# Champii/raiko

Measured on AMD Instinct MI355X. Metric: proven RISC-V cycles/sec, higher is better.
Workload: dtype u32 (BabyBear Montgomery)

## Files before the change

### include/raiko_hip.h

```cpp
#ifndef RAIKO_HIP_H
#define RAIKO_HIP_H
#include <stddef.h>
#include <stdint.h>

#ifdef __cplusplus
extern "C" {
#endif

typedef enum {
    RK_OK = 0,
    RK_ERR_INVALID = -1,
    RK_ERR_HIP = -2,
    RK_ERR_NOMEM = -3,
    RK_ERR_NODEVICE = -4,
    RK_ERR_CAPACITY = -5,
    RK_ERR_INTERNAL = -6,
    RK_ERR_VERIFY = -7,
    RK_ERR_CALLBACK = -8
} rk_status;

typedef struct rk_ctx rk_ctx;

int rk_abi_version(void);
const char* rk_strerror(int status);
// ... 179 lines not shown

typedef struct {
    int device;
    int inflight;
    int upload_ahead;
    int verify;
    const int* devices;
    int n_devices;
    const rk_verify_opts* verify_opts;
    const rk_params* params;
} rk_session_opts;
int rk_prove_session(const rk_session_opts* opts, const rk_segment* segs, size_t n, uint32_t* const* h_seals,
                     const size_t* seal_capacity_words, size_t* seal_words, size_t* failed_index);
typedef struct rk_stream rk_stream;
int rk_stream_open(const rk_session_opts* opts, rk_stream** out);
int rk_stream_submit(rk_stream* stream, const rk_segment* seg, uint32_t* h_seal, size_t seal_capacity_words, size_t* seal_words);
int rk_stream_wait(rk_stream* stream, size_t max_pending, size_t* finished_prefix);
int rk_stream_close(rk_stream* stream, size_t* failed_index);
const char* rk_session_last_error(int device);
int rk_session_last_proven(int device, size_t* count);
int rk_session_release(void);
int rk_code_cache_configure(int device, size_t max_bytes);
int rk_code_cache_stats(int device, uint64_t* hits, uint64_t* misses, uint64_t* bytes);

typedef struct rk_comm rk_comm;
#define RK_COMM_ID_BYTES 128
int rk_comm_unique_id(uint8_t id[RK_COMM_ID_BYTES]);
int rk_comm_create(const uint8_t id[RK_COMM_ID_BYTES], int rank, int world, int device, rk_comm** out);
int rk_comm_destroy(rk_comm* comm);
const char* rk_comm_last_error(rk_comm* comm);
int rk_gather_seals(rk_comm* comm, const uint32_t* const* h_local_seals, const size_t* local_words, size_t n_local, size_t n_total,
                    uint32_t* const* h_out, const size_t* out_capacity, size_t* out_words);
int rk_gather_unpack(const uint32_t* all_lens, const uint32_t* all_payload, int world, size_t per_rank, size_t max_len, size_t n_total,
                     uint32_t* const* h_out, const size_t* out_capacity, size_t* out_words);

typedef struct rk_exec rk_exec;
enum { RK_ECALL_HALT = 0, RK_ECALL_READ = 1, RK_ECALL_COMMIT = 2 };
enum { RK_EXIT_HALTED = 0, RK_EXIT_SYSTEM_SPLIT = 2 };
typedef struct {
    uint32_t struct_size;
    uint32_t segment_limit_po2;
    uint64_t session_limit;
    const uint32_t* input_words;
    size_t n_input_words;
    uint32_t record_trace;
    uint32_t profile;
// ... 334 lines not shown
```

### provers/hip/driver/src/ffi.rs

```rust
#![allow(non_camel_case_types)]
#![allow(clippy::missing_safety_doc)]
use std::os::raw::{c_char, c_int, c_void};
pub const RK_ECALL_HALT: c_int = 0;
pub const RK_ECALL_READ: c_int = 1;
pub const RK_ECALL_COMMIT: c_int = 2;

pub const RK_EXIT_HALTED: c_int = 0;
pub const RK_EXIT_SYSTEM_SPLIT: c_int = 2;

pub type rk_status = c_int;
pub const RK_OK: rk_status = 0;
pub const RK_ERR_INVALID: rk_status = -1;
pub const RK_ERR_HIP: rk_status = -2;
pub const RK_ERR_NOMEM: rk_status = -3;
pub const RK_ERR_NODEVICE: rk_status = -4;
pub const RK_ERR_CAPACITY: rk_status = -5;
pub const RK_ERR_INTERNAL: rk_status = -6;
pub const RK_ERR_VERIFY: rk_status = -7;
pub const RK_ERR_CALLBACK: rk_status = -8;

pub type rk_preset = c_int;
pub const RK_PRESET_RISC0: rk_preset = 0;
pub const RK_PRESET_SP1: rk_preset = 1;

// ... 218 lines not shown
#[repr(C)]
#[derive(Clone, Copy)]
pub struct rk_verify_opts {
    pub p2_rc_ext: *const u32,
    pub p2_rc_int: *const u32,
    pub p2_diag: *const u32,
    pub poly_ext: Option<rk_poly_ext_fn>,
    pub user: *mut c_void,
    pub program: *const rk_program,
    pub params: *const rk_params,
}

#[repr(C)]
#[derive(Clone, Copy)]
pub struct rk_session_opts {
    pub device: c_int,
    pub inflight: c_int,
    pub upload_ahead: c_int,
    pub verify: c_int,
    pub devices: *const c_int,
    pub n_devices: c_int,
    pub verify_opts: *const rk_verify_opts,
    pub params: *const rk_params,
}

#[repr(C)]
#[derive(Clone, Copy)]
pub struct rk_exec_opts {
    pub struct_size: u32,
    pub segment_limit_po2: u32,
    pub session_limit: u64,
    pub input_words: *const u32,
    pub n_input_words: usize,
    pub record_trace: u32,
    pub profile: u32,
}

#[repr(C)]
#[derive(Clone, Copy)]
pub struct rk_exec_summary {
    pub total_cycles: u64,
    pub n_segments: u32,
    pub exit_code: u32,
    pub journal_bytes: usize,
    pub input_words_read: usize,
    pub status: c_int,
// ... 287 lines not shown
    pub fn rk_program_create(steps: *const rk_poly_step, n_steps: usize, ret: u32, taps: *const rk_taps, out: *mut *mut rk_program) -> c_int;
    pub fn rk_program_destroy(prog: *mut rk_program) -> c_int;
    pub fn rk_program_get_info(prog: *const rk_program, out: *mut rk_program_info) -> c_int;
    pub fn rk_program_eval_check(prog: *const rk_program, view: *const rk_circuit_view, poly_mix: *const u32, d_check: *mut u32) -> c_int;
    pub fn rk_program_compile(prog: *mut rk_program, ctx: *mut rk_ctx) -> c_int;
    pub fn rk_program_source(prog: *const rk_program, out: *mut c_char, capacity: usize, length: *mut usize) -> c_int;
    pub fn rk_program_poly_ext(prog: *const rk_program, ext_w: u32, poly_mix: *const u32, eval_u_ext: *const u32, n_taps: usize, globals: *const u32, n_globals: u32, mix: *const u32, n_mix: u32, out_ext: *mut u32) -> c_int;
    pub fn rk_prove_segment(ctx: *mut rk_ctx, seg: *const rk_segment, h_seal: *mut u32, seal_capacity_words: usize, seal_words: *mut usize) -> c_int;
    pub fn rk_verify_segment(pub_: *const rk_segment, seal: *const u32, seal_words: usize) -> c_int;
    pub fn rk_verify_segment_ex(pub_: *const rk_segment, opts: *const rk_verify_opts, seal: *const u32, seal_words: usize) -> c_int;
    pub fn rk_seal_bound_words(seg: *const rk_segment) -> usize;
    pub fn rk_seal_bound_words_for(seg: *const rk_segment, queries: u32) -> usize;
    pub fn rk_seal_bound_words_params(seg: *const rk_segment, params: *const rk_params) -> usize;
    pub fn rk_prove_session(opts: *const rk_session_opts, segs: *const rk_segment, n: usize, h_seals: *const *mut u32, seal_capacity_words: *const usize, seal_words: *mut usize, failed_index: *mut usize) -> c_int;
    pub fn rk_stream_open(opts: *const rk_session_opts, out: *mut *mut rk_stream) -> c_int;
    pub fn rk_stream_submit(stream: *mut rk_stream, seg: *const rk_segment, h_seal: *mut u32, seal_capacity_words: usize, seal_words: *mut usize) -> c_int;
    pub fn rk_stream_wait(stream: *mut rk_stream, max_pending: usize, finished_prefix: *mut usize) -> c_int;
    pub fn rk_stream_close(stream: *mut rk_stream, failed_index: *mut usize) -> c_int;
    pub fn rk_session_last_error(device: c_int) -> *const c_char;
    pub fn rk_session_last_proven(device: c_int, count: *mut usize) -> c_int;
    pub fn rk_session_release() -> c_int;
    pub fn rk_code_cache_configure(device: c_int, max_bytes: usize) -> c_int;
    pub fn rk_code_cache_stats(device: c_int, hits: *mut u64, misses: *mut u64, bytes: *mut u64) -> c_int;
    pub fn rk_comm_unique_id(id: *mut u8) -> c_int;
    pub fn rk_comm_create(id: *const u8, rank: c_int, world: c_int, device: c_int, out: *mut *mut rk_comm) -> c_int;
    pub fn rk_comm_destroy(comm: *mut rk_comm) -> c_int;
    pub fn rk_comm_last_error(comm: *mut rk_comm) -> *const c_char;
    pub fn rk_gather_seals(comm: *mut rk_comm, h_local_seals: *const *const u32, local_words: *const usize, n_local: usize, n_total: usize, h_out: *const *mut u32, out_capacity: *const usize, out_words: *mut usize) -> c_int;
    pub fn rk_gather_unpack(all_lens: *const u32, all_payload: *const u32, world: c_int, per_rank: usize, max_len: usize, n_total: usize, h_out: *const *mut u32, out_capacity: *const usize, out_words: *mut usize) -> c_int;
    pub fn rk_exec_elf(elf: *const u8, elf_bytes: usize, opts: *const rk_exec_opts, out: *mut *mut rk_exec) -> c_int;
    pub fn rk_exec_open(elf: *const u8, elf_bytes: usize, opts: *const rk_exec_opts, out: *mut *mut rk_exec) -> c_int;
    pub fn rk_exec_next_segment(ex: *mut rk_exec, more: *mut c_int) -> c_int;
    pub fn rk_exec_summary_get(ex: *const rk_exec, out: *mut rk_exec_summary) -> c_int;
    pub fn rk_exec_segment_get(ex: *const rk_exec, index: u32, out: *mut rk_exec_segment) -> c_int;
    pub fn rk_exec_journal(ex: *const rk_exec, out: *mut u8, capacity: usize, len: *mut usize) -> c_int;
    pub fn rk_exec_profile(ex: *const rk_exec, pcs: *mut u32, cycles: *mut u64, capacity: usize, n: *mut usize) -> c_int;
    pub fn rk_exec_witness(ex: *const rk_exec, index: u32, code: *mut u32, data: *mut u32) -> c_int;
    pub fn rk_exec_lookup_tables(ex: *const rk_exec, index: u32, range_table: *mut u32, program_table: *mut u32, program_rows: *mut usize) -> c_int;
    pub fn rk_exec_witness_device(ctx: *mut rk_ctx, ex: *const rk_exec, index: u32, d_code: *mut u32, d_data: *mut u32) -> c_int;
    pub fn rk_exec_witness_device_rows(ctx: *mut rk_ctx, ex: *const rk_exec, index: u32, d_rows: *mut u32) -> c_int;
    pub fn rk_exec_registers(ex: *const rk_exec, index: u32, start: *mut u32, end: *mut u32) -> c_int;
    pub fn rk_exec_ecalls(ex: *const rk_exec, index: u32, out: *mut u32, capacity: usize, n: *mut usize) -> c_int;
    pub fn rk_exec_rv32_sizes(ex: *const rk_exec, index: u32, program_rows: *mut usize) -> c_int;
    pub fn rk_exec_rv32_shard_device(ctx: *mut rk_ctx, ex: *const rk_exec, index: u32, d_cpu: *mut u32, d_program: *mut u32, program_rows: usize, d_register: *mut u32, d_byte: *mut u32, d_range: *mut u32) -> c_int;
    pub fn rk_exec_rv32cf_shard_device(ctx: *mut rk_ctx, ex: *const rk_exec, index: u32, d_cpu: *mut u32, d_program: *mut u32, program_rows: usize, d_register: *mut u32, d_byte: *mut u32, d_range: *mut u32, d_shift: *mut u32) -> c_int;
    pub fn rk_exec_rv32im_sizes(ex: *const rk_exec, index: u32, muldiv_rows: *mut usize) -> c_int;
// ... 80 lines not shown
```

### raiko_amd/_lib.py

```python
import ctypes as C
import os

_HERE = os.path.dirname(os.path.abspath(__file__))
LIB_PATH = os.environ.get("RAIKO_HIP_LIB") or os.path.join(_HERE, "libraiko_hip.so")


class HipLibraryError(RuntimeError):
    pass


class RkError(RuntimeError):
    def __init__(self, status, detail=""):
        self.status = status
        super().__init__(f"libraiko_hip status {status}: {detail}")


u32p = C.POINTER(C.c_uint32)


class RkTaps(C.Structure):
    _fields_ = [
        ("group_size", C.c_uint32 * 3),
        ("n_regs", C.c_uint32),
        ("reg_group", u32p),
# ... 63 lines not shown

class RkVerifyOpts(C.Structure):
    _fields_ = [("p2_rc_ext", u32p), ("p2_rc_int", u32p), ("p2_diag", u32p), ("poly_ext", POLY_EXT_FN),
                ("user", C.c_void_p), ("program", C.c_void_p), ("params", C.POINTER(RkParams))]


class RkSessionOpts(C.Structure):
    _fields_ = [("device", C.c_int), ("inflight", C.c_int), ("upload_ahead", C.c_int), ("verify", C.c_int),
                ("devices", C.POINTER(C.c_int)), ("n_devices", C.c_int), ("verify_opts", C.POINTER(RkVerifyOpts)),
                ("params", C.POINTER(RkParams))]


RK_ERR_INVALID = -1
RK_ERR_CAPACITY = -5
RK_ERR_INTERNAL = -6
RK_ERR_VERIFY = -7
RK_ERR_CALLBACK = -8


class RkKernelStat(C.Structure):
    _fields_ = [("launches", C.c_uint64), ("ms", C.c_double), ("bytes", C.c_double)]


KCLASS_COUNT = 5


class RkTiming(C.Structure):
    _fields_ = [(n, C.c_float) for n in ("ntt", "hash", "deep", "fri", "query", "total", "circuit")]


class RkFriReduceSizeInfo(C.Structure):
    _fields_ = [(n, C.c_uint32) for n in ("n_rounds", "n_slots", "fold_width", "path_width", "reduce_width", "chip_width", "fold_log_height",
                                          "path_log_height", "reduce_log_height", "chip_log_height")] + \
               [(n, C.c_uint64) for n in ("fold_rows", "path_rows", "reduce_rows", "chip_rows", "rows_per_query", "fold_publics_words",
                                          "fold_records_words", "reduce_publics_words", "inputs_words")]


class RkFriOpenSizeInfo(C.Structure):
    _fields_ = [(n, C.c_uint32) for n in ("n_rounds", "n_slots", "n_groups", "n_batches", "log_pmax", "log_kmax", "fold_width", "path_width",
                                          "reduce_width", "ipath_width", "chip_width", "state_width", "fold_log_height", "path_log_height",
                                          "reduce_log_height", "ipath_log_height", "chip_log_height", "state_log_height")] + \
               [(n, C.c_uint64) for n in ("fold_rows", "path_rows", "reduce_rows", "ipath_rows", "chip_rows", "state_rows", "rows_per_query",
                                          "fold_publics_words", "fold_records_words", "reduce_publics_words", "inputs_words", "roots_words",
                                          "paths_words")]


# ... 50 lines not shown
class RkExecSummary(C.Structure):
    _fields_ = [("total_cycles", C.c_uint64), ("n_segments", C.c_uint32), ("exit_code", C.c_uint32),
                ("journal_bytes", C.c_size_t), ("input_words_read", C.c_size_t), ("status", C.c_int)]


class RkExecSegment(C.Structure):
    _fields_ = [("index", C.c_uint32), ("po2", C.c_uint32), ("cycles", C.c_uint64), ("start_pc", C.c_uint32),
                ("end_pc", C.c_uint32), ("exit", C.c_uint32), ("pre_state", C.c_uint32 * 8), ("post_state", C.c_uint32 * 8)]


_vp, _sz, _u32 = C.c_void_p, C.c_size_t, C.c_uint32
SYMBOLS = {
    "rk_prove_session": (C.c_int, [C.POINTER(RkSessionOpts), C.POINTER(RkSegment), _sz, C.POINTER(u32p), C.POINTER(_sz),
                                   C.POINTER(_sz), C.POINTER(_sz)]),
    "rk_session_last_error": (C.c_char_p, [C.c_int]),
    "rk_stream_open": (C.c_int, [C.POINTER(RkSessionOpts), C.POINTER(C.c_void_p)]),
    "rk_stream_submit": (C.c_int, [C.c_void_p, C.POINTER(RkSegment), u32p, C.c_size_t, C.POINTER(C.c_size_t)]),
    "rk_stream_wait": (C.c_int, [C.c_void_p, C.c_size_t, C.POINTER(C.c_size_t)]),
    "rk_stream_close": (C.c_int, [C.c_void_p, C.POINTER(C.c_size_t)]),
    "rk_session_release": (C.c_int, []),
    "rk_session_last_proven": (C.c_int, [C.c_int, C.POINTER(C.c_size_t)]),
    "rk_code_cache_configure": (C.c_int, [C.c_int, C.c_size_t]),
    "rk_code_cache_stats": (C.c_int, [C.c_int, C.POINTER(C.c_uint64), C.POINTER(C.c_uint64), C.POINTER(C.c_uint64)]),
    "rk_abi_version": (C.c_int, []),
    "rk_strerror": (C.c_char_p, [C.c_int]),
    "rk_last_error": (C.c_char_p, [_vp]),
    "rk_device_count": (C.c_int, [C.POINTER(C.c_int)]),
    "rk_ctx_create": (C.c_int, [C.c_int, _vp, C.POINTER(_vp)]),
    "rk_ctx_destroy": (C.c_int, [_vp]),
    "rk_sync": (C.c_int, [_vp]),
    "rk_alloc": (C.c_int, [_vp, _sz, C.POINTER(_vp)]),
    "rk_free": (C.c_int, [_vp, _vp]),
    "rk_h2d": (C.c_int, [_vp, _vp, _vp, _sz]),
    "rk_d2h": (C.c_int, [_vp, _vp, _vp, _sz]),
    "rk_set_poseidon2_params": (C.c_int, [_vp, u32p, u32p, u32p]),
    "rk_batch_interpolate_ntt": (C.c_int, [_vp, _vp, _sz, _sz]),
    "rk_batch_evaluate_ntt": (C.c_int, [_vp, _vp, _sz, _sz, _u32]),
    "rk_zk_shift": (C.c_int, [_vp, _vp, _sz, _sz]),
    "rk_batch_expand_into_evaluate_ntt": (C.c_int, [_vp, _vp, _vp, _sz, _sz, _u32]),
    "rk_batch_bit_reverse": (C.c_int, [_vp, _vp, _sz, _sz]),
    "rk_hash_rows": (C.c_int, [_vp, _vp, _vp, _sz, _sz]),
    "rk_hash_fold": (C.c_int, [_vp, _vp, _sz, _sz]),
    "rk_batch_evaluate_any": (C.c_int, [_vp, _vp, _sz, _sz, u32p, u32p, _sz, u32p]),
    "rk_mix_poly_coeffs": (C.c_int, [_vp, _vp, u32p, u32p, _vp, u32p, _sz, _sz]),
    "rk_eltwise_add_elem": (C.c_int, [_vp, _vp, _vp, _vp, _sz]),
    "rk_eltwise_sum_extelem": (C.c_int, [_vp, _vp, _vp, _sz, _sz]),
# ... 205 lines not shown
```

### raiko_amd/csrc/code_cache.hip

```cpp
#include "internal.hpp"

#include <cstdlib>
#include <list>
#include <mutex>
#include <random>

namespace rk {

namespace {

constexpr unsigned FP_CHUNK = 4096;
constexpr unsigned FP_TPB = 256;
constexpr unsigned FP_PER_LANE = FP_CHUNK / FP_TPB;
constexpr size_t FP_MAX_CHUNKS = (size_t)1 << 16;
constexpr unsigned FP_MAX_BLOCKS = 1024;
constexpr unsigned FP_PART = 8;

__global__ __launch_bounds__(FP_TPB) void code_fingerprint_kernel(uint32_t* __restrict__ part, const uint32_t* __restrict__ m,
                                                                  size_t words, const uint32_t* __restrict__ ta,
                                                                  const uint32_t* __restrict__ tb, uint32_t wm, int vec) {
    const unsigned t = threadIdx.x;
    uint32_t a[FP_PER_LANE][4];
#pragma unroll
    for (unsigned q = 0; q < 4; q++)
// ... 38 lines not shown
        tot = bb::add(tot, bb::mul(s, bb::Ext{{bv.x, bv.y, bv.z, bv.w}}, wm));
    }
    __shared__ uint32_t red[FP_TPB][5];
#pragma unroll
    for (unsigned c = 0; c < 4; c++) red[t][c] = tot.c[c];
    red[t][4] = bad;
    __syncthreads();
    for (unsigned h = FP_TPB / 2; h > 0; h >>= 1) {
        if (t < h) {
#pragma unroll
            for (unsigned c = 0; c < 4; c++) red[t][c] = bb::add(red[t][c], red[t + h][c]);
            red[t][4] |= red[t + h][4];
        }
        __syncthreads();
    }
    if (t < 5) part[(size_t)blockIdx.x * FP_PART + t] = red[0][t];
}

struct DevCache {
    std::mutex mu;
    std::list<std::shared_ptr<CodeEntry>> lru;
    size_t bytes = 0, max_bytes = 0;
    uint64_t hits = 0, misses = 0;
    uint32_t* d_tables = nullptr;
};

std::mutex g_mu;
std::map<int, DevCache*>* g_caches = nullptr;

size_t default_bytes() {
    static const size_t v = [] {
        const char* e = std::getenv("RK_CODE_CACHE_BYTES");
        if (e && *e) return (size_t)std::strtoull(e, nullptr, 0);
        return (size_t)2 << 30;
    }();
    return v;
}

DevCache* cache_of(int device) {
    std::lock_guard<std::mutex> l(g_mu);
    if (!g_caches) g_caches = new std::map<int, DevCache*>();
    DevCache*& c = (*g_caches)[device];
    if (!c) {
        c = new DevCache();
        c->max_bytes = default_bytes();
    }
// ... 78 lines not shown
    for (int i = 0; i < 4; i++) fp[i] = sum.c[i];
    *canonical = bad == 0;
    return RK_OK;
}

CodeKey code_key(const rk_ctx* ctx, uint32_t po2, uint32_t cols, uint32_t queries, const uint32_t fp[4]) {
    CodeKey key{};
    std::memcpy(key.fp, fp, sizeof key.fp);
    key.po2 = po2;
    key.cols = cols;
    key.blowup_log2 = ctx->sys.blowup_log2;
    key.queries = queries;
    key.root27m = ctx->sys.root27m;
    key.shiftm = ctx->sys.shiftm;
    const p2::Any& kc = ctx->h_p2;
    std::vector<uint32_t> inst{bb::encode((uint32_t)kc.kind), bb::encode(kc.pad_free ? 1u : 0u)};
    inst.insert(inst.end(), kc.rc_ext(), kc.rc_ext() + 8 * kc.cells());
    inst.insert(inst.end(), kc.rc_int(), kc.rc_int() + kc.rounds_partial());
    inst.insert(inst.end(), kc.diag(), kc.diag() + kc.cells());
    kc.hash_elems(inst.data(), inst.size(), key.p2);
    return key;
}

std::shared_ptr<CodeEntry> code_cache_lookup(int device, const CodeKey& key) {
    DevCache* c = cache_of(device);
    std::lock_guard<std::mutex> l(c->mu);
    for (auto it = c->lru.begin(); it != c->lru.end(); ++it) {
        if (!((*it)->key == key)) continue;
        c->lru.splice(c->lru.begin(), c->lru, it);
        c->hits++;
        return c->lru.front();
    }
    c->misses++;
    return nullptr;
}

std::shared_ptr<CodeEntry> code_cache_new_entry(int device, const CodeKey& key, size_t coeff_bytes, size_t eval_bytes, size_t node_bytes) {
    auto e = std::make_shared<CodeEntry>();
    e->key = key;
    e->device = device;
    e->bytes = coeff_bytes + eval_bytes + node_bytes;
    if (hipMalloc((void**)&e->coeffs, coeff_bytes) != hipSuccess || hipMalloc((void**)&e->evaluated, eval_bytes) != hipSuccess ||
        hipMalloc((void**)&e->nodes, node_bytes) != hipSuccess || hipEventCreateWithFlags(&e->ready, hipEventDisableTiming) != hipSuccess) {
        (void)hipGetLastError();
        return nullptr;
    }
    return e;
}

void code_cache_insert(const std::shared_ptr<CodeEntry>& e) {
    DevCache* c = cache_of(e->device);
    std::vector<std::shared_ptr<CodeEntry>> evicted;
    {
        std::lock_guard<std::mutex> l(c->mu);
        if (c->max_bytes == 0 || e->bytes > c->max_bytes) return;
        for (const auto& o : c->lru)
            if (o->key == e->key) return;
        while (!c->lru.empty() && c->bytes + e->bytes > c->max_bytes) {
            c->bytes -= c->lru.back()->bytes;
            evicted.push_back(std::move(c->lru.back()));
            c->lru.pop_back();
        }
        c->lru.push_front(e);
        c->bytes += e->bytes;
    }
}

void code_cache_release() {
    std::vector<DevCache*> all;
    {
        std::lock_guard<std::mutex> l(g_mu);
        if (g_caches)
            for (auto& kv : *g_caches) all.push_back(kv.second);
    }
    for (DevCache* c : all) {
        std::list<std::shared_ptr<CodeEntry>> gone;
        std::lock_guard<std::mutex> l(c->mu);
        gone.swap(c->lru);
        c->bytes = 0;
    }
}

}

extern "C" {

int rk_code_cache_configure(int device, size_t max_bytes) {
    RK_GUARD_BEGIN
    if (device < 0) return RK_ERR_INVALID;
    rk::DevCache* c = rk::cache_of(device);
    std::vector<std::shared_ptr<rk::CodeEntry>> evicted;
    std::lock_guard<std::mutex> l(c->mu);
    c->max_bytes = max_bytes;
    while (!c->lru.empty() && c->bytes > max_bytes) {
        c->bytes -= c->lru.back()->bytes;
        evicted.push_back(std::move(c->lru.back()));
        c->lru.pop_back();
    }
    return RK_OK;
    RK_GUARD_END
}

int rk_code_cache_stats(int device, uint64_t* hits, uint64_t* misses, uint64_t* bytes) {
    RK_GUARD_BEGIN
    if (device < 0) return RK_ERR_INVALID;
    rk::DevCache* c = rk::cache_of(device);
    std::lock_guard<std::mutex> l(c->mu);
    if (hits) *hits = c->hits;
    if (misses) *misses = c->misses;
    if (bytes) *bytes = c->bytes;
    return RK_OK;
    RK_GUARD_END
}

}
```

### raiko_amd/csrc/internal.hpp

```cpp
#pragma once
#include <hip/hip_runtime.h>

#include <cstring>
#include <map>
#include <memory>
#include <mutex>
#include <new>
#include <string>
#include <unordered_map>
#include <vector>

#include "../../include/raiko_hip.h"
#include "taps.hpp"
#include "bb.hpp"
#include "ntt_core.hpp"
#include "poseidon2_core.hpp"
#include "params.hpp"

struct rk_ctx {
    int device = 0;
    hipStream_t stream = nullptr;
    bool own_stream = false;
    std::string last_error;

// ... 10 lines not shown
    size_t pool_limit = (size_t)24 << 30;

    void* d_scratch = nullptr;
    size_t scratch_bytes = 0;
    void* h_ring = nullptr;
    size_t h_ring_at = 0;
    bool h_ring_failed = false;

    rk_timing timing{};
    rk_p3_timing p3_timing{};
    std::vector<hipEvent_t> stage_events;

    bool ktime_on = false;
    struct KRec {
        hipEvent_t a, b;
        int cls;
        double bytes;
    };
    std::vector<KRec> krecs;
    size_t krec_used = 0;
    double k_ms[RK_KCLASS_COUNT] = {0};
    double k_bytes[RK_KCLASS_COUNT] = {0};
    uint64_t k_launches[RK_KCLASS_COUNT] = {0};
};

#define RK_HIP_TRY(ctx, expr)                                                                   \
    do {                                                                                        \
        hipError_t _e = (expr);                                                                 \
        if (_e != hipSuccess) {                                                                 \
            (ctx)->last_error = std::string(#expr) + ": " + hipGetErrorString(_e);              \
            return RK_ERR_HIP;                                                                  \
        }                                                                                       \
    } while (0)
#define RK_GUARD_BEGIN try {
#define RK_GUARD_END                                   \
    }                                                  \
    catch (const std::bad_alloc&) { return RK_ERR_NOMEM; } \
    catch (...) { return RK_ERR_INTERNAL; }
#define RK_TRY(expr)                \
    do {                            \
        int _s = (expr);            \
        if (_s != RK_OK) return _s; \
    } while (0)

static inline bool is_pow2(size_t n) { return n && !(n & (n - 1)); }
static inline unsigned log2u(size_t n) {
// ... 161 lines not shown
    uint32_t fp[4];
    uint32_t po2, cols, blowup_log2, queries;
    uint32_t root27m, shiftm;
    uint32_t p2[8];
    bool operator==(const CodeKey& o) const { return std::memcmp(this, &o, sizeof(CodeKey)) == 0; }
};
struct CodeEntry {
    CodeKey key{};
    int device = 0;
    uint32_t* coeffs = nullptr;
    uint32_t* evaluated = nullptr;
    uint32_t* nodes = nullptr;
    std::vector<uint32_t> top;
    hipEvent_t ready = nullptr;
    size_t bytes = 0;
    CodeEntry() = default;
    CodeEntry(const CodeEntry&) = delete;
    CodeEntry& operator=(const CodeEntry&) = delete;
    ~CodeEntry();
};
bool code_cache_usable(int device, size_t words, size_t entry_bytes);
int code_fingerprint(rk_ctx* ctx, const uint32_t* d_src, size_t words, uint32_t fp[4], bool* canonical);
CodeKey code_key(const rk_ctx* ctx, uint32_t po2, uint32_t cols, uint32_t queries, const uint32_t fp[4]);
std::shared_ptr<CodeEntry> code_cache_lookup(int device, const CodeKey& key);
std::shared_ptr<CodeEntry> code_cache_new_entry(int device, const CodeKey& key, size_t coeff_bytes, size_t eval_bytes, size_t node_bytes);
void code_cache_insert(const std::shared_ptr<CodeEntry>& e);
void code_cache_release();

}
```

### raiko_amd/csrc/prover.hip

```cpp
#include "segment_host.hpp"

#include <algorithm>
#include <cstring>
#include <memory>

namespace {

using bb::Ext;
using rk::d2h_sync;
using rk::DevBuf;

struct Transcript {
    p2::Rng rng;
    std::vector<uint32_t> proof;
    explicit Transcript(const p2::Any* kc) : rng(kc) {}
    void write(const uint32_t* w, size_t n) { proof.insert(proof.end(), w, w + n); }
    void commit(const uint32_t* digest) { rng.mix(digest); }
    uint32_t random_elem() { return rng.random_elem(); }
    Ext random_ext() { return rng.random_ext(); }
    uint32_t random_bits(unsigned bits) { return rng.random_bits(bits); }
};

struct MerkleDev {
    size_t rows = 0, cols = 0, layers = 0, top_layer = 0, top_size = 1;
// ... 277 lines not shown
        } else {
            RK_TRY(raw[g].alloc(ctx, words * 4));
            RK_HIP_TRY(ctx, hipMemcpyAsync(raw[g].p, src, words * 4, hipMemcpyHostToDevice, ctx->stream));
            d_raw[g] = raw[g].u32();
        }
        from = d_raw[g];
        return dst.alloc(ctx, words * 4);
    }
    int commit_loaded(PolyGroup& pg, const uint32_t* from, size_t count) {
        sw.start("ntt");
        RK_TRY(rk::ntt_reverse_from(ctx, pg.coeffs.u32(), from ? from : pg.coeffs.u32(), N, count, true));
        RK_TRY(pg.build(ctx, count, N));
        sw.stop(&ctx->timing.ntt);
        sw.start("hash");
        RK_TRY(pg.merkle.build(ctx, pg.evaluated.u32(), D, count, QUERIES));
        sw.stop(&ctx->timing.hash);
        return pg.merkle.commit(ctx, iop);
    }
    int commit_group(int g, PolyGroup& pg, const uint32_t* trace, size_t count, bool preloaded = false) {
        const uint32_t* from = nullptr;
        if (!preloaded) RK_TRY(load_group(g, pg.coeffs, trace, count * N, from));
        return commit_loaded(pg, from, count);
    }
    int commit_code() {
        PolyGroup& pg = groups[1];
        const size_t count = taps.group_size[1], words = count * N;
        const size_t coeff_bytes = words * 4, eval_bytes = count * D * 4, node_bytes = 2 * D * p2::OUT * 4;
        if (!rk::code_cache_usable(ctx->device, words, coeff_bytes + eval_bytes + node_bytes))
            return commit_group(1, pg, seg->group[1], count);
        const uint32_t* src = seg->group[1];
        if (!seg->on_device) {
            RK_TRY(raw[1].alloc(ctx, words * 4));
            RK_HIP_TRY(ctx, hipMemcpyAsync(raw[1].p, src, words * 4, hipMemcpyHostToDevice, ctx->stream));
            src = raw[1].u32();
        }
        if (hook_accum) d_raw[1] = src;
        uint32_t fp[4];
        bool canonical = false;
        RK_TRY(rk::code_fingerprint(ctx, src, words, fp, &canonical));
        const rk::CodeKey key = canonical ? rk::code_key(ctx, seg->po2, (uint32_t)count, (uint32_t)QUERIES, fp) : rk::CodeKey{};
        std::shared_ptr<rk::CodeEntry> hit = canonical ? rk::code_cache_lookup(ctx->device, key) : nullptr;
        pg.count = count;
        pg.size = N;
        if (hit) {
            code_ref = hit;
            RK_HIP_TRY(ctx, hipStreamWaitEvent(ctx->stream, hit->ready, 0));
            pg.coeffs.adopt(ctx, hit->coeffs);
            pg.evaluated.adopt(ctx, hit->evaluated);
            pg.merkle.shape(hit->evaluated, D, count, QUERIES);
            pg.merkle.nodes.adopt(ctx, hit->nodes);
            pg.merkle.top = hit->top;
            pg.merkle.commit_top(iop);
        } else {
            std::shared_ptr<rk::CodeEntry> fresh;
            if (canonical) fresh = rk::code_cache_new_entry(ctx->device, key, coeff_bytes, eval_bytes, node_bytes);
            if (fresh) {
                code_ref = fresh;
                pg.coeffs.adopt(ctx, fresh->coeffs);
                pg.evaluated.adopt(ctx, fresh->evaluated);
                pg.merkle.nodes.adopt(ctx, fresh->nodes);
            } else {
                RK_TRY(pg.coeffs.alloc(ctx, words * 4));
            }
            RK_TRY(commit_loaded(pg, src, count));
            if (fresh) {
                fresh->top = pg.merkle.top;
                RK_HIP_TRY(ctx, hipEventRecord(fresh->ready, ctx->stream));
                rk::code_cache_insert(fresh);
            }
        }
        if (!hook_accum) raw[1].release();
        return RK_OK;
    }

    int accumulate() {
// ... 226 lines not shown
                jobs.push_back(OpenJob{&rounds[k]->merkle, pos, &oround[k]});
            }
            RK_TRY(open_many(ctx, jobs));
        }
        for (size_t q = 0; q < QUERIES; q++) {
            for (int g = 0; g < 3; g++) write_opening(iop, groups[g].merkle, og[g], q);
            write_opening(iop, check.merkle, ocheck, q);
            for (size_t k = 0; k < rounds.size(); k++) write_opening(iop, rounds[k]->merkle, oround[k], q);
        }
        sw.stop(&ctx->timing.query);
        return RK_OK;
    }
};

int prove_segment(rk_ctx* ctx, const rk_segment* seg, std::vector<uint32_t>& seal) {
    const rk_taps& taps = seg->taps;
    RK_TRY(rk::check_taps(taps));
    const rk::Shape shape = ctx->sys.shape();
    if (!rk::shape_ok(shape) || seg->po2 < 1 || seg->po2 + shape.blowup_log2 > ntt::LAMBDA) return RK_ERR_INVALID;
    const rk_circuit_hooks* hooks = seg->hooks;
    const bool hook_accum = hooks && hooks->accumulate, hook_check = hooks && (hooks->eval_check || hooks->program);
    for (int g = 0; g < 3; g++) {
        if (taps.group_size[g] == 0) return RK_ERR_INVALID;
        if (!seg->group[g] && !(g == 0 && hook_accum)) return RK_ERR_INVALID;
    }
    if ((!seg->check && !hook_check) || (seg->n_globals && !seg->globals)) return RK_ERR_INVALID;
    if (seg->n_accum_mix > (1u << 16)) return RK_ERR_INVALID;
    for (uint32_t c = 0; c < taps.n_combos; c++)
        if (rk::combo_taps(taps, c) > ((size_t)1 << seg->po2)) return RK_ERR_INVALID;
    SegmentRun run(ctx, seg, shape);
    return run.prove(seal);
}

}

extern "C" {

size_t rk_seal_bound_words(const rk_segment* seg) { return rk::seal_bound_words(seg); }
size_t rk_seal_bound_words_for(const rk_segment* seg, uint32_t queries) { return rk::seal_bound_words(seg, (size_t)queries); }
size_t rk_seal_bound_words_params(const rk_segment* seg, const rk_params* params) {
    if (!params || params->struct_size != sizeof(rk_params)) return 0;
    return rk::seal_bound_words(seg, rk::Shape{params->queries, params->blowup_log2, params->fri_fold_log2, params->fri_min_degree,
                                               params->pow_bits});
}

int rk_prove_segment(rk_ctx* ctx, const rk_segment* seg, uint32_t* h_seal, size_t cap, size_t* seal_words) {
    RK_GUARD_BEGIN
// ... 17 lines not shown
```

### raiko_amd/csrc/session.hip

```cpp
#include <condition_variable>
#include <deque>
#include <map>
#include <memory>
#include <mutex>
#include <thread>
#include <vector>

#include <cstdlib>

#include "inflight.hpp"
#include "internal.hpp"

namespace {

int logical_devices() {
    const char* e = std::getenv("RK_TEST_LOGICAL_DEVICES");
    if (!e || !*e) return 0;
    const int k = std::atoi(e);
    return k > 0 && k <= 64 ? k : 0;
}
int physical_of(int device, int n_gpus) { return logical_devices() > 0 && n_gpus > 0 ? device % n_gpus : device; }

struct RingSlot {
    void* group[3] = {nullptr, nullptr, nullptr};
    void* check = nullptr;
    size_t words[4] = {0, 0, 0, 0};
};

void free_slot(rk_ctx* up, RingSlot* s) {
    for (int g = 0; g < 3; g++) {
        if (s->group[g]) (void)rk_free(up, s->group[g]);
        s->group[g] = nullptr;
    }
    if (s->check) (void)rk_free(up, s->check);
    s->check = nullptr;
    for (auto& w : s->words) w = 0;
}

struct DevicePool : rk::CtxPool {
    int device = 0;
    std::vector<RingSlot*> ring;
    std::string last_error;
    int physical = 0;
    size_t last_proven = 0;
    bool ktime_on = false;
    void clear() {
        for (RingSlot* s : ring) {
            free_slot(uploader, s);
            delete s;
        }
        ring.clear();
        rk::CtxPool::clear();
    }
    ~DevicePool() { clear(); }
};

std::mutex g_mu;
std::map<int, std::shared_ptr<DevicePool>> g_pools;

struct FreeSlots {
    std::mutex mu;
    std::deque<RingSlot*> slots;
};

bool needs_staging(const rk_segment& s) { return s.on_device == 0; }
bool hook_accum(const rk_segment& s) { return s.hooks && s.hooks->accumulate; }
bool hook_check(const rk_segment& s) { return s.hooks && (s.hooks->eval_check || s.hooks->program); }

int stage_segment(rk_ctx* up, const rk_segment& seg, unsigned blowup_log2, RingSlot* slot) {
    const size_t rows = (size_t)1 << seg.po2;
    const size_t want[4] = {hook_accum(seg) ? 0 : rows * seg.taps.group_size[0], rows * seg.taps.group_size[1],
                            rows * seg.taps.group_size[2], hook_check(seg) ? 0 : (rows * 4) << blowup_log2};
    int st = RK_OK;
    if (want[0] != slot->words[0] || want[1] != slot->words[1] || want[2] != slot->words[2] || want[3] != slot->words[3]) {
        free_slot(up, slot);
        for (int g = 0; g < 3 && st == RK_OK; g++)
            if (want[g]) st = rk_alloc(up, want[g] * 4, &slot->group[g]);
        if (st == RK_OK && want[3]) st = rk_alloc(up, want[3] * 4, &slot->check);
        if (st == RK_OK)
            for (int k = 0; k < 4; k++) slot->words[k] = want[k];
    }
    for (int g = 0; g < 3 && st == RK_OK; g++) {
        if (!want[g]) continue;
        st = seg.group[g] ? rk_h2d(up, slot->group[g], seg.group[g], want[g] * 4) : RK_ERR_INVALID;
    }
    if (st == RK_OK && want[3]) st = seg.check ? rk_h2d(up, slot->check, seg.check, want[3] * 4) : RK_ERR_INVALID;
    if (st == RK_OK) st = rk_sync(up);
    return st;
}

int prove_session(const rk_session_opts* opts, const rk_segment* segs, size_t n, uint32_t* const* h_seals,
                  const size_t* seal_capacity_words, size_t* seal_words, size_t* failed_index) {
    if (failed_index) *failed_index = (size_t)-1;
    if (!opts || (n && (!segs || !h_seals || !seal_capacity_words || !seal_words))) return RK_ERR_INVALID;
    if (!rk::inflight::opts_ok(opts->inflight, opts->upload_ahead, opts->n_devices, opts->devices)) return RK_ERR_INVALID;
    std::vector<int> devices;
    if (!rk::inflight::device_list(opts->device, opts->devices, opts->n_devices, &devices)) return RK_ERR_INVALID;
    if (n == 0) return RK_OK;
    int n_gpus = 0;
    if (hipGetDeviceCount(&n_gpus) != hipSuccess || n_gpus <= 0) return RK_ERR_NODEVICE;
    const int n_visible = logical_devices() > 0 ? logical_devices() : n_gpus;
    for (int d : devices)
        if (d < 0 || d >= n_visible) return RK_ERR_INVALID;

    std::vector<std::shared_ptr<DevicePool>> pools;
    {
        std::lock_guard<std::mutex> l(g_mu);
        for (int d : devices) {
            auto& sp = g_pools[d];
// ... 51 lines not shown
        const size_t had = pool->slots.size();
        RK_TRY(pool->ensure(pool->physical, workers, &prm, key));
        for (size_t j = had; pool->ktime_on && j < pool->slots.size(); j++) (void)rk_set_kernel_timing(pool->slots[j].ctx, 1);
        if (any_host) RK_TRY(pool->ensure_uploader(pool->physical));
        for (size_t k = 0; k < pool->ring.size() && k < n_slots; k++) free_slots[d].slots.push_back(pool->ring[k]);
    }

    rk::inflight::Calls<RingSlot*> calls;
    calls.stage = [&](size_t d, size_t i, RingSlot** out) -> int {
        if (!needs_staging(segs[i])) return RK_OK;
        RingSlot* slot = nullptr;
        {
            std::lock_guard<std::mutex> l(free_slots[d].mu);
            if (!free_slots[d].slots.empty()) {
                slot = free_slots[d].slots.front();
                free_slots[d].slots.pop_front();
            } else {
                auto fresh = std::make_unique<RingSlot>();
                pools[d]->ring.push_back(fresh.get());
                slot = fresh.release();
            }
        }
        *out = slot;
        return stage_segment(pools[d]->uploader, segs[i], prm.blowup_log2, slot);
    };
    calls.prove = [&](size_t d, size_t w, size_t i, RingSlot*& slot) -> int {
        rk_segment seg = segs[i];
        if (slot) {
            seg.on_device = 2;
            for (int g = 0; g < 3; g++) seg.group[g] = (const uint32_t*)slot->group[g];
            seg.check = (const uint32_t*)slot->check;
        }
        return rk_prove_segment(pools[d]->slots[w].ctx, &seg, h_seals[i], seal_capacity_words[i], &seal_words[i]);
    };
    calls.release = [&](size_t d, RingSlot*& slot) {
        if (!slot) return;
        std::lock_guard<std::mutex> l(free_slots[d].mu);
        free_slots[d].slots.push_back(slot);
    };
    calls.verify = [&](size_t i) -> int { return rk_verify_segment_ex(&segs[i], verify_opts, h_seals[i], seal_words[i]); };
    calls.error_text = [&](size_t d, int w) { return rk_last_error(w < 0 ? pools[d]->uploader : pools[d]->slots[(size_t)w].ctx); };

    const size_t n_verifiers = rk::inflight::verifier_threads(opts->verify, devices.size(), n, std::thread::hardware_concurrency());
    rk::inflight::Pipeline<RingSlot*> run(n, std::move(owner), devices.size(), workers, n_slots, n_verifiers, std::move(calls));
    const int status = run.run();
    for (size_t d = 0; d < devices.size(); d++) pools[d]->last_proven = run.devs[d].proven;
    if (status != RK_OK) {
        if (failed_index) *failed_index = run.failed;
        std::lock_guard<std::mutex> l(g_mu);
        for (auto& p : pools) p->last_error = run.detail;
    }
    return status;
}

}

// ... 232 lines not shown
```

### raiko_amd/hal.py

```python
import ctypes as C
from typing import Optional, Sequence

import numpy as np

from . import _lib
from .segment import Segment, TapSet


def _u32p(a: np.ndarray):
    return a.ctypes.data_as(_lib.u32p)


class DeviceBuffer:

    def __init__(self, hal: "HipHal", words: int):
        self.hal = hal
        self.words = int(words)
        ptr = C.c_void_p()
        _lib.check(hal._ctx, hal._lib.rk_alloc(hal._ctx, self.words * 4, C.byref(ptr)))
        self.ptr = ptr.value

    def size(self) -> int:
        return self.words

# ... 388 lines not shown
    return p


def session_last_proven(device: int) -> int:
    n = C.c_size_t(0)
    _lib.check(None, _lib.load().rk_session_last_proven(device, C.byref(n)))
    return int(n.value)


def session_release():
    _lib.check(None, _lib.load().rk_session_release())


def code_cache_configure(device: int, max_bytes: int):
    _lib.check(None, _lib.load().rk_code_cache_configure(device, max_bytes))


def code_cache_stats(device: int) -> dict:
    h, m, b = C.c_uint64(0), C.c_uint64(0), C.c_uint64(0)
    _lib.check(None, _lib.load().rk_code_cache_stats(device, C.byref(h), C.byref(m), C.byref(b)))
    return {"hits": int(h.value), "misses": int(m.value), "bytes": int(b.value)}


def session_set_kernel_timing(device: int, enabled: bool):
    lib = _lib.load()
    _lib.check(None, lib.rk_session_set_kernel_timing(device, 1 if enabled else 0))


def session_kernel_stats(device: int) -> dict:
    lib = _lib.load()
    out = {}
    for k in range(_lib.KCLASS_COUNT):
        st = _lib.RkKernelStat()
        _lib.check(None, lib.rk_session_kernel_stats(device, k, C.byref(st)))
        out[lib.rk_kernel_class_name(k).decode()] = {"launches": int(st.launches), "ms": float(st.ms), "bytes": float(st.bytes)}
    return out


def mmcs_verify(heights, widths, index: int, rows, path, root, params=None) -> int:
    lib = _lib.load()
    h = np.ascontiguousarray(heights, dtype=np.uint32)
    w = np.ascontiguousarray(widths, dtype=np.uint32)
    r = np.ascontiguousarray(rows, dtype=np.uint32)
    p = np.ascontiguousarray(path, dtype=np.uint32).reshape(-1)
    if p.size == 0:
        p = np.zeros(8, dtype=np.uint32)
# ... 108 lines not shown
```

Measured before the change: 50.73 million.

## Skip code-group upload when host content matches a known cached program

Adds a host-side store of recently seen code-group contents, keyed by fingerprint. During staging, a background thread compares the incoming code group against it (sparse probe, then full memcmp) while the other groups upload. On a match the H2D copy, fingerprint kernel and commitment are skipped and the device code cache entry is borrowed directly. The cost is extra host memory (up to 1 GiB by default), a per-segment thread spawn and memcmp, and a sync D2H copy the first time a program is inserted.

New measurement: 50.82 million (median of 3 runs). Within noise of the previous version (+0.2%).

```diff
diff --git a/include/raiko_hip.h b/include/raiko_hip.h
--- a/include/raiko_hip.h
+++ b/include/raiko_hip.h
@@ -225,6 +225,13 @@
 int rk_session_release(void);
 int rk_code_cache_configure(int device, size_t max_bytes);
 int rk_code_cache_stats(int device, uint64_t* hits, uint64_t* misses, uint64_t* bytes);
+typedef struct {
+    uint64_t code_skipped;
+    uint64_t code_uploaded;
+    uint64_t h2d_bytes;
+    uint64_t compare_ns;
+} rk_code_upload_stat;
+int rk_code_upload_stats(int device, rk_code_upload_stat* out);
 
 typedef struct rk_comm rk_comm;
 #define RK_COMM_ID_BYTES 128
diff --git a/provers/hip/driver/src/ffi.rs b/provers/hip/driver/src/ffi.rs
--- a/provers/hip/driver/src/ffi.rs
+++ b/provers/hip/driver/src/ffi.rs
@@ -264,6 +264,15 @@
     pub n_devices: c_int,
     pub verify_opts: *const rk_verify_opts,
     pub params: *const rk_params,
+}
+
+#[repr(C)]
+#[derive(Clone, Copy)]
+pub struct rk_code_upload_stat {
+    pub code_skipped: u64,
+    pub code_uploaded: u64,
+    pub h2d_bytes: u64,
+    pub compare_ns: u64,
 }
 
 #[repr(C)]
@@ -597,6 +606,7 @@
     pub fn rk_session_release() -> c_int;
     pub fn rk_code_cache_configure(device: c_int, max_bytes: usize) -> c_int;
     pub fn rk_code_cache_stats(device: c_int, hits: *mut u64, misses: *mut u64, bytes: *mut u64) -> c_int;
+    pub fn rk_code_upload_stats(device: c_int, out: *mut rk_code_upload_stat) -> c_int;
     pub fn rk_comm_unique_id(id: *mut u8) -> c_int;
     pub fn rk_comm_create(id: *const u8, rank: c_int, world: c_int, device: c_int, out: *mut *mut rk_comm) -> c_int;
     pub fn rk_comm_destroy(comm: *mut rk_comm) -> c_int;
diff --git a/raiko_amd/_lib.py b/raiko_amd/_lib.py
--- a/raiko_amd/_lib.py
+++ b/raiko_amd/_lib.py
@@ -109,6 +109,11 @@
     _fields_ = [("launches", C.c_uint64), ("ms", C.c_double), ("bytes", C.c_double)]
 
 
+class RkCodeUploadStat(C.Structure):
+    _fields_ = [("code_skipped", C.c_uint64), ("code_uploaded", C.c_uint64), ("h2d_bytes", C.c_uint64),
+                ("compare_ns", C.c_uint64)]
+
+
 KCLASS_COUNT = 5
 
 
@@ -205,6 +210,7 @@
     "rk_session_last_proven": (C.c_int, [C.c_int, C.POINTER(C.c_size_t)]),
     "rk_code_cache_configure": (C.c_int, [C.c_int, C.c_size_t]),
     "rk_code_cache_stats": (C.c_int, [C.c_int, C.POINTER(C.c_uint64), C.POINTER(C.c_uint64), C.POINTER(C.c_uint64)]),
+    "rk_code_upload_stats": (C.c_int, [C.c_int, C.POINTER(RkCodeUploadStat)]),
     "rk_abi_version": (C.c_int, []),
     "rk_strerror": (C.c_char_p, [C.c_int]),
     "rk_last_error": (C.c_char_p, [_vp]),
diff --git a/raiko_amd/csrc/code_cache.hip b/raiko_amd/csrc/code_cache.hip
--- a/raiko_amd/csrc/code_cache.hip
+++ b/raiko_amd/csrc/code_cache.hip
@@ -1,4 +1,5 @@
 #include "internal.hpp"
+#include "code_known.hpp"
 
 #include <cstdlib>
 #include <list>
@@ -84,6 +85,7 @@
     std::list<std::shared_ptr<CodeEntry>> lru;
     size_t bytes = 0, max_bytes = 0;
     uint64_t hits = 0, misses = 0;
+    rk_code_upload_stat up{};
     uint32_t* d_tables = nullptr;
 };
 
@@ -208,7 +210,7 @@
     return key;
 }
 
-std::shared_ptr<CodeEntry> code_cache_lookup(int device, const CodeKey& key) {
+std::shared_ptr<CodeEntry> code_cache_lookup(int device, const CodeKey& key, bool count_miss) {
     DevCache* c = cache_of(device);
     std::lock_guard<std::mutex> l(c->mu);
     for (auto it = c->lru.begin(); it != c->lru.end(); ++it) {
@@ -217,7 +219,7 @@
         c->hits++;
         return c->lru.front();
     }
-    c->misses++;
+    if (count_miss) c->misses++;
     return nullptr;
 }
 
@@ -252,7 +254,17 @@
     }
 }
 
+void code_upload_count(int device, uint64_t skipped, uint64_t uploaded, uint64_t h2d_bytes, uint64_t compare_ns) {
+    DevCache* c = cache_of(device);
+    std::lock_guard<std::mutex> l(c->mu);
+    c->up.code_skipped += skipped;
+    c->up.code_uploaded += uploaded;
+    c->up.h2d_bytes += h2d_bytes;
+    c->up.compare_ns += compare_ns;
+}
+
 void code_cache_release() {
+    code_known().clear();
     std::vector<DevCache*> all;
     {
         std::lock_guard<std::mutex> l(g_mu);
@@ -299,4 +311,14 @@
     RK_GUARD_END
 }
 
-}
+int rk_code_upload_stats(int device, rk_code_upload_stat* out) {
+    RK_GUARD_BEGIN
+    if (device < 0 || !out) return RK_ERR_INVALID;
+    rk::DevCache* c = rk::cache_of(device);
+    std::lock_guard<std::mutex> l(c->mu);
+    *out = c->up;
+    return RK_OK;
+    RK_GUARD_END
+}
+
+}
diff --git a/raiko_amd/csrc/code_known.hpp b/raiko_amd/csrc/code_known.hpp
--- /dev/null
+++ b/raiko_amd/csrc/code_known.hpp
@@ -0,0 +1,144 @@
+#pragma once
+#include <algorithm>
+#include <cstdint>
+#include <cstdlib>
+#include <cstring>
+#include <list>
+#include <memory>
+#include <mutex>
+#include <new>
+#include <vector>
+
+namespace rk {
+
+class CodeKnown {
+public:
+    struct Record {
+        size_t words = 0;
+        uint32_t domain = 0;
+        uint32_t fp[4] = {0, 0, 0, 0};
+        bool canonical = false;
+        std::unique_ptr<uint32_t[]> copy;
+    };
+    static constexpr size_t MAX_RECORDS = 8;
+    static constexpr size_t PROBES = 16;
+
+    explicit CodeKnown(size_t max_bytes = (size_t)1 << 30, size_t max_records = MAX_RECORDS)
+        : max_bytes_(max_bytes), max_records_(max_records) {}
+
+    void configure(size_t max_bytes, size_t max_records) {
+        std::vector<std::shared_ptr<const Record>> gone;
+        std::lock_guard<std::mutex> l(mu_);
+        max_bytes_ = max_bytes;
+        max_records_ = max_records;
+        trim(0, 0, gone);
+    }
+
+    static bool probe_differs(const uint32_t* a, const uint32_t* b, size_t words) {
+        if (words == 0) return false;
+        const size_t step = words / PROBES ? words / PROBES : 1;
+        for (size_t i = 0; i < words; i += step)
+            if (a[i] != b[i]) return true;
+        return a[words - 1] != b[words - 1];
+    }
+
+    bool lookup(const uint32_t* h, size_t words, uint32_t domain, uint32_t fp[4]) {
+        if (!h) return false;
+        std::vector<std::shared_ptr<const Record>> cand;
+        {
+            std::lock_guard<std::mutex> l(mu_);
+            for (const auto& r : lru_)
+                if (r->words == words && r->domain == domain) cand.push_back(r);
+        }
+        for (const auto& r : cand) {
+            if (probe_differs(h, r->copy.get(), words)) continue;
+            if (words && std::memcmp(h, r->copy.get(), words * sizeof(uint32_t)) != 0) continue;
+            std::memcpy(fp, r->fp, sizeof r->fp);
+            std::lock_guard<std::mutex> l(mu_);
+            auto it = std::find(lru_.begin(), lru_.end(), r);
+            if (it != lru_.end()) lru_.splice(lru_.begin(), lru_, it);
+            hits_++;
+            return true;
+        }
+        std::lock_guard<std::mutex> l(mu_);
+        misses_++;
+        return false;
+    }
+
+    bool has(const uint32_t fp[4], size_t words, uint32_t domain) {
+        std::lock_guard<std::mutex> l(mu_);
+        return find(fp, words, domain) != lru_.end();
+    }
+
+    template <class Fill>
+    bool insert(const uint32_t fp[4], size_t words, uint32_t domain, bool canonical, Fill&& fill) {
+        if (!canonical) return false;
+        const size_t bytes = words * sizeof(uint32_t);
+        {
+            std::lock_guard<std::mutex> l(mu_);
+            if (max_records_ == 0 || bytes > max_bytes_) return false;
+            if (find(fp, words, domain) != lru_.end()) return false;
+        }
+        auto r = std::make_shared<Record>();
+        r->words = words;
+        r->domain = domain;
+        std::memcpy(r->fp, fp, sizeof r->fp);
+        r->canonical = true;
+        r->copy.reset(new (std::nothrow) uint32_t[words ? words : 1]);
+        if (!r->copy || !fill(r->copy.get())) return false;
+        std::vector<std::shared_ptr<const Record>> gone;
+        std::lock_guard<std::mutex> l(mu_);
+        if (max_records_ == 0 || bytes > max_bytes_) return false;
+        if (find(fp, words, domain) != lru_.end()) return false;
+        trim(bytes, 1, gone);
+        lru_.push_front(std::move(r));
+        bytes_ += bytes;
+        return true;
+    }
+
+    void clear() {
+        std::list<std::shared_ptr<const Record>> gone;
+        std::lock_guard<std::mutex> l(mu_);
+        gone.swap(lru_);
+        bytes_ = 0;
+    }
+
+    struct Stats {
+        size_t records, bytes;
+        uint64_t hits, misses;
+    };
+    Stats stats() {
+        std::lock_guard<std::mutex> l(mu_);
+        return Stats{lru_.size(), bytes_, hits_, misses_};
+    }
+
+private:
+    using List = std::list<std::shared_ptr<const Record>>;
+    List::iterator find(const uint32_t fp[4], size_t words, uint32_t domain) {
+        return std::find_if(lru_.begin(), lru_.end(), [&](const std::shared_ptr<const Record>& r) {
+            return r->words == words && r->domain == domain && std::memcmp(r->fp, fp, sizeof r->fp) == 0;
+        });
+    }
+    void trim(size_t bytes, size_t more, std::vector<std::shared_ptr<const Record>>& gone) {
+        while (!lru_.empty() && (bytes_ + bytes > max_bytes_ || lru_.size() + more > max_records_)) {
+            bytes_ -= lru_.back()->words * sizeof(uint32_t);
+            gone.push_back(std::move(lru_.back()));
+            lru_.pop_back();
+        }
+    }
+
+    std::mutex mu_;
+    List lru_;
+    size_t bytes_ = 0, max_bytes_, max_records_;
+    uint64_t hits_ = 0, misses_ = 0;
+};
+
+inline CodeKnown& code_known() {
+    static CodeKnown* t = [] {
+        const char* e = std::getenv("RK_CODE_KNOWN_BYTES");
+        return new CodeKnown(e && *e ? (size_t)std::strtoull(e, nullptr, 0) : (size_t)1 << 30);
+    }();
+    return *t;
+}
+
+}
diff --git a/raiko_amd/csrc/internal.hpp b/raiko_amd/csrc/internal.hpp
--- a/raiko_amd/csrc/internal.hpp
+++ b/raiko_amd/csrc/internal.hpp
@@ -56,6 +56,12 @@
     double k_ms[RK_KCLASS_COUNT] = {0};
     double k_bytes[RK_KCLASS_COUNT] = {0};
     uint64_t k_launches[RK_KCLASS_COUNT] = {0};
+
+    struct CodeHint {
+        const uint32_t* host = nullptr;
+        bool skipped = false;
+        uint32_t fp[4] = {0, 0, 0, 0};
+    } code_hint;
 };
 
 #define RK_HIP_TRY(ctx, expr)                                                                   \
@@ -263,9 +269,10 @@
 bool code_cache_usable(int device, size_t words, size_t entry_bytes);
 int code_fingerprint(rk_ctx* ctx, const uint32_t* d_src, size_t words, uint32_t fp[4], bool* canonical);
 CodeKey code_key(const rk_ctx* ctx, uint32_t po2, uint32_t cols, uint32_t queries, const uint32_t fp[4]);
-std::shared_ptr<CodeEntry> code_cache_lookup(int device, const CodeKey& key);
+std::shared_ptr<CodeEntry> code_cache_lookup(int device, const CodeKey& key, bool count_miss = true);
 std::shared_ptr<CodeEntry> code_cache_new_entry(int device, const CodeKey& key, size_t coeff_bytes, size_t eval_bytes, size_t node_bytes);
 void code_cache_insert(const std::shared_ptr<CodeEntry>& e);
 void code_cache_release();
+void code_upload_count(int device, uint64_t skipped, uint64_t uploaded, uint64_t h2d_bytes, uint64_t compare_ns);
 
 }
diff --git a/raiko_amd/csrc/prover.hip b/raiko_amd/csrc/prover.hip
--- a/raiko_amd/csrc/prover.hip
+++ b/raiko_amd/csrc/prover.hip
@@ -1,4 +1,5 @@
 #include "segment_host.hpp"
+#include "code_known.hpp"
 
 #include <algorithm>
 #include <cstring>
@@ -323,35 +324,60 @@
         if (!preloaded) RK_TRY(load_group(g, pg.coeffs, trace, count * N, from));
         return commit_loaded(pg, from, count);
     }
+    int borrow_code(PolyGroup& pg, const std::shared_ptr<rk::CodeEntry>& hit, size_t count) {
+        code_ref = hit;
+        RK_HIP_TRY(ctx, hipStreamWaitEvent(ctx->stream, hit->ready, 0));
+        pg.coeffs.adopt(ctx, hit->coeffs);
+        pg.evaluated.adopt(ctx, hit->evaluated);
+        pg.merkle.shape(hit->evaluated, D, count, QUERIES);
+        pg.merkle.nodes.adopt(ctx, hit->nodes);
+        pg.merkle.top = hit->top;
+        pg.merkle.commit_top(iop);
+        return RK_OK;
+    }
     int commit_code() {
         PolyGroup& pg = groups[1];
         const size_t count = taps.group_size[1], words = count * N;
         const size_t coeff_bytes = words * 4, eval_bytes = count * D * 4, node_bytes = 2 * D * p2::OUT * 4;
-        if (!rk::code_cache_usable(ctx->device, words, coeff_bytes + eval_bytes + node_bytes))
-            return commit_group(1, pg, seg->group[1], count);
+        const rk_ctx::CodeHint hint = seg->on_device == 2 ? ctx->code_hint : rk_ctx::CodeHint{};
+        const uint32_t* host = seg->on_device ? hint.host : seg->group[1];
+        const bool usable = rk::code_cache_usable(ctx->device, words, coeff_bytes + eval_bytes + node_bytes);
+        if (!usable && !hint.skipped) return commit_group(1, pg, seg->group[1], count);
+        pg.count = count;
+        pg.size = N;
+        uint32_t fp[4];
+        bool known = hint.skipped;
+        if (known) std::memcpy(fp, hint.fp, sizeof fp);
+        else if (!seg->on_device && !hook_accum) known = rk::code_known().lookup(host, words, ctx->sys.wm, fp);
+        if (known && usable) {
+            const rk::CodeKey key = rk::code_key(ctx, seg->po2, (uint32_t)count, (uint32_t)QUERIES, fp);
+            if (std::shared_ptr<rk::CodeEntry> hit = rk::code_cache_lookup(ctx->device, key, false)) {
+                rk::code_upload_count(ctx->device, 1, 0, 0, 0);
+                return borrow_code(pg, hit, count);
+            }
+        }
         const uint32_t* src = seg->group[1];
-        if (!seg->on_device) {
+        if (!seg->on_device || hint.skipped) {
             RK_TRY(raw[1].alloc(ctx, words * 4));
-            RK_HIP_TRY(ctx, hipMemcpyAsync(raw[1].p, src, words * 4, hipMemcpyHostToDevice, ctx->stream));
+            RK_HIP_TRY(ctx, hipMemcpyAsync(raw[1].p, host, words * 4, hipMemcpyHostToDevice, ctx->stream));
+            rk::code_upload_count(ctx->device, 0, 1, words * 4, 0);
             src = raw[1].u32();
         }
+        if (!usable) {
+            RK_TRY(pg.coeffs.alloc(ctx, words * 4));
+            RK_TRY(commit_loaded(pg, src, count));
+            raw[1].release();
+            return RK_OK;
+        }
         if (hook_accum) d_raw[1] = src;
-        uint32_t fp[4];
         bool canonical = false;
         RK_TRY(rk::code_fingerprint(ctx, src, words, fp, &canonical));
+        if (canonical && host && !rk::code_known().has(fp, words, ctx->sys.wm))
+            (void)rk::code_known().insert(fp, words, ctx->sys.wm, true, [&](uint32_t* dst) { return rk::d2h_sync(ctx, dst, src, words * 4) == RK_OK; });
         const rk::CodeKey key = canonical ? rk::code_key(ctx, seg->po2, (uint32_t)count, (uint32_t)QUERIES, fp) : rk::CodeKey{};
         std::shared_ptr<rk::CodeEntry> hit = canonical ? rk::code_cache_lookup(ctx->device, key) : nullptr;
-        pg.count = count;
-        pg.size = N;
         if (hit) {
-            code_ref = hit;
-            RK_HIP_TRY(ctx, hipStreamWaitEvent(ctx->stream, hit->ready, 0));
-            pg.coeffs.adopt(ctx, hit->coeffs);
-            pg.evaluated.adopt(ctx, hit->evaluated);
-            pg.merkle.shape(hit->evaluated, D, count, QUERIES);
-            pg.merkle.nodes.adopt(ctx, hit->nodes);
-            pg.merkle.top = hit->top;
-            pg.merkle.commit_top(iop);
+            RK_TRY(borrow_code(pg, hit, count));
         } else {
             std::shared_ptr<rk::CodeEntry> fresh;
             if (canonical) fresh = rk::code_cache_new_entry(ctx->device, key, coeff_bytes, eval_bytes, node_bytes);
@@ -624,7 +650,8 @@
     const bool hook_accum = hooks && hooks->accumulate, hook_check = hooks && (hooks->eval_check || hooks->program);
     for (int g = 0; g < 3; g++) {
         if (taps.group_size[g] == 0) return RK_ERR_INVALID;
-        if (!seg->group[g] && !(g == 0 && hook_accum)) return RK_ERR_INVALID;
+        const bool code_known = g == 1 && seg->on_device == 2 && ctx->code_hint.skipped && ctx->code_hint.host && !hook_accum;
+        if (!seg->group[g] && !(g == 0 && hook_accum) && !code_known) return RK_ERR_INVALID;
     }
     if ((!seg->check && !hook_check) || (seg->n_globals && !seg->globals)) return RK_ERR_INVALID;
     if (seg->n_accum_mix > (1u << 16)) return RK_ERR_INVALID;
diff --git a/raiko_amd/csrc/session.hip b/raiko_amd/csrc/session.hip
--- a/raiko_amd/csrc/session.hip
+++ b/raiko_amd/csrc/session.hip
@@ -1,3 +1,4 @@
+#include <chrono>
 #include <condition_variable>
 #include <deque>
 #include <map>
@@ -8,6 +9,7 @@
 
 #include <cstdlib>
 
+#include "code_known.hpp"
 #include "inflight.hpp"
 #include "internal.hpp"
 
@@ -25,16 +27,18 @@
     void* group[3] = {nullptr, nullptr, nullptr};
     void* check = nullptr;
     size_t words[4] = {0, 0, 0, 0};
+    bool code_skipped = false;
+    uint32_t code_fp[4] = {0, 0, 0, 0};
+    void*& buf(int k) { return k < 3 ? group[k] : check; }
 };
 
 void free_slot(rk_ctx* up, RingSlot* s) {
-    for (int g = 0; g < 3; g++) {
-        if (s->group[g]) (void)rk_free(up, s->group[g]);
-        s->group[g] = nullptr;
-    }
-    if (s->check) (void)rk_free(up, s->check);
-    s->check = nullptr;
-    for (auto& w : s->words) w = 0;
+    for (int k = 0; k < 4; k++) {
+        if (s->buf(k)) (void)rk_free(up, s->buf(k));
+        s->buf(k) = nullptr;
+        s->words[k] = 0;
+    }
+    s->code_skipped = false;
 }
 
 struct DevicePool : rk::CtxPool {
@@ -67,24 +71,50 @@
 bool hook_accum(const rk_segment& s) { return s.hooks && s.hooks->accumulate; }
 bool hook_check(const rk_segment& s) { return s.hooks && (s.hooks->eval_check || s.hooks->program); }
 
-int stage_segment(rk_ctx* up, const rk_segment& seg, unsigned blowup_log2, RingSlot* slot) {
+int stage_segment(rk_ctx* up, const rk_segment& seg, unsigned blowup_log2, uint32_t fp_domain, RingSlot* slot) {
     const size_t rows = (size_t)1 << seg.po2;
     const size_t want[4] = {hook_accum(seg) ? 0 : rows * seg.taps.group_size[0], rows * seg.taps.group_size[1],
                             rows * seg.taps.group_size[2], hook_check(seg) ? 0 : (rows * 4) << blowup_log2};
+    const uint32_t* const from[4] = {seg.group[0], seg.group[1], seg.group[2], seg.check};
+    const size_t entry_bytes = want[1] * 4 + ((want[1] * 4) << blowup_log2) + ((2 * rows * p2::OUT * 4) << blowup_log2);
+    const bool look = !hook_accum(seg) && seg.group[1] && rk::code_cache_usable(up->device, want[1], entry_bytes);
+    slot->code_skipped = false;
+    bool found = false;
+    uint64_t compare_ns = 0;
+    std::thread compare;
+    if (look)
+        compare = std::thread([&] {
+            const auto t0 = std::chrono::steady_clock::now();
+            try {
+                found = rk::code_known().lookup(seg.group[1], want[1], fp_domain, slot->code_fp);
+            } catch (...) {
+                found = false;
+            }
+            compare_ns = (uint64_t)std::chrono::duration_cast<std::chrono::nanoseconds>(std::chrono::steady_clock::now() - t0).count();
+        });
     int st = RK_OK;
-    if (want[0] != slot->words[0] || want[1] != slot->words[1] || want[2] != slot->words[2] || want[3] != slot->words[3]) {
-        free_slot(up, slot);
-        for (int g = 0; g < 3 && st == RK_OK; g++)
-            if (want[g]) st = rk_alloc(up, want[g] * 4, &slot->group[g]);
-        if (st == RK_OK && want[3]) st = rk_alloc(up, want[3] * 4, &slot->check);
-        if (st == RK_OK)
-            for (int k = 0; k < 4; k++) slot->words[k] = want[k];
-    }
-    for (int g = 0; g < 3 && st == RK_OK; g++) {
-        if (!want[g]) continue;
-        st = seg.group[g] ? rk_h2d(up, slot->group[g], seg.group[g], want[g] * 4) : RK_ERR_INVALID;
-    }
-    if (st == RK_OK && want[3]) st = seg.check ? rk_h2d(up, slot->check, seg.check, want[3] * 4) : RK_ERR_INVALID;
+    uint64_t sent = 0;
+    auto send = [&](int k) -> int {
+        if (!want[k]) return RK_OK;
+        if (!from[k]) return RK_ERR_INVALID;
+        if (want[k] != slot->words[k]) {
+            if (slot->buf(k)) (void)rk_free(up, slot->buf(k));
+            slot->buf(k) = nullptr;
+            slot->words[k] = 0;
+            RK_TRY(rk_alloc(up, want[k] * 4, &slot->buf(k)));
+            slot->words[k] = want[k];
+        }
+        sent += want[k] * 4;
+        return rk_h2d(up, slot->buf(k), from[k], want[k] * 4);
+    };
+    for (int k : {0, 2, 3})
+        if (st == RK_OK) st = send(k);
+    if (compare.joinable()) compare.join();
+    if (st == RK_OK) {
+        if (found) slot->code_skipped = true;
+        else if ((st = send(1)) == RK_OK) rk::code_upload_count(up->device, 0, want[1] ? 1 : 0, 0, 0);
+    }
+    rk::code_upload_count(up->device, 0, 0, sent, compare_ns);
     if (st == RK_OK) st = rk_sync(up);
     return st;
 }
@@ -182,7 +212,7 @@
             }
         }
         *out = slot;
-        return stage_segment(pools[d]->uploader, segs[i], prm.blowup_log2, slot);
+        return stage_segment(pools[d]->uploader, segs[i], prm.blowup_log2, pools[d]->slots[0].ctx->sys.wm, slot);
     };
     calls.prove = [&](size_t d, size_t w, size_t i, RingSlot*& slot) -> int {
         rk_segment seg = segs[i];
@@ -191,7 +221,16 @@
             for (int g = 0; g < 3; g++) seg.group[g] = (const uint32_t*)slot->group[g];
             seg.check = (const uint32_t*)slot->check;
         }
-        return rk_prove_segment(pools[d]->slots[w].ctx, &seg, h_seals[i], seal_capacity_words[i], &seal_words[i]);
+        rk_ctx* ctx = pools[d]->slots[w].ctx;
+        if (slot) {
+            ctx->code_hint.host = segs[i].group[1];
+            ctx->code_hint.skipped = slot->code_skipped;
+            std::memcpy(ctx->code_hint.fp, slot->code_fp, sizeof slot->code_fp);
+            if (slot->code_skipped) seg.group[1] = nullptr;
+        }
+        const int st = rk_prove_segment(ctx, &seg, h_seals[i], seal_capacity_words[i], &seal_words[i]);
+        ctx->code_hint = rk_ctx::CodeHint{};
+        return st;
     };
     calls.release = [&](size_t d, RingSlot*& slot) {
         if (!slot) return;
diff --git a/raiko_amd/hal.py b/raiko_amd/hal.py
--- a/raiko_amd/hal.py
+++ b/raiko_amd/hal.py
@@ -434,6 +434,12 @@
     return {"hits": int(h.value), "misses": int(m.value), "bytes": int(b.value)}
 
 
+def code_upload_stats(device: int) -> dict:
+    st = _lib.RkCodeUploadStat()
+    _lib.check(None, _lib.load().rk_code_upload_stats(device, C.byref(st)))
+    return {n: int(getattr(st, n)) for n, _ in st._fields_}
+
+
 def session_set_kernel_timing(device: int, enabled: bool):
     lib = _lib.load()
     _lib.check(None, lib.rk_session_set_kernel_timing(device, 1 if enabled else 0))
```
